# malak29/video-text-detection-system

Measured on AMD Instinct MI355X. Metric: frames/sec (detect+recognize) @720p, 1/2/4/8 MI355X; box IoU vs CPU ref, higher is better.
Workload: dtype f16

## Files before the change

video-text-detection-system_amd/csrc/conv_halo.hip:

```cpp
#include <cstdio>
#include <cstdlib>
#include "vtd_common.h"

namespace {

struct HaloParams {
    const half_t* in;
    const half_t* wgt;
    const float* bias;
    const half_t* res;
    half_t* out;
    int n, h, w, cin, cout;
    int in_hp, in_wp, in_ring, out_hp, out_wp, out_ring, res_hp, res_wp, res_ring;
    int tiles_x, tiles_y, tiles_n, relu;
    unsigned long long* stamps;
    int dbg;
};

template <int N>
__device__ __forceinline__ void hl_wait_vmcnt() {
    asm volatile("s_waitcnt vmcnt(%0)" ::"n"(N) : "memory");
}

template <int BN, int TW>
__global__ __launch_bounds__((BN / 64) * 256) void conv_halo_kernel(const HaloParams p) {
    constexpr int WN = BN / 64, NW = 4 * WN, NT = NW * 64, TH = 256 / TW;
    constexpr int HWD = TW + 2, HROWS = (TH + 2) * HWD, HPIECES = (HROWS + 7) / 8, HBYTES = HPIECES * 1024;
    constexpr int HPW = (HPIECES + NW - 1) / NW;
    constexpr int HPS = (HPW + 7) / 8;
    constexpr int BSTAGE = BN * 128, BPW = BN / 8 / NW;
    constexpr int EPI_ROW = BN * 4 + 16;
    static_assert(BPW == 2, "two weight pieces per wave and K-step");
    extern __shared__ __attribute__((aligned(16))) char smem[];

    const int nchunks = p.cin >> 6;
    const int hb_stride = nchunks > 1 ? HBYTES : 0;
    char* const bring = smem + (nchunks > 1 ? 2 : 1) * HBYTES;

    const int nblk = gridDim.x, b = blockIdx.x;
    const int q8 = nblk >> 3, r8 = nblk & 7, xcd = b & 7;
    int tile = (xcd < r8 ? xcd * (q8 + 1) : r8 * (q8 + 1) + (xcd - r8) * q8) + (b >> 3);
    const int tn = tile % p.tiles_n;
    tile /= p.tiles_n;
    const int tx = tile % p.tiles_x;
    tile /= p.tiles_x;
    const int ty = tile % p.tiles_y;
    const int img = tile / p.tiles_y;
    const int y0 = ty * TH, x0 = tx * TW, n0 = tn * BN;

    const int tid = threadIdx.x, lane = tid & 63;
    const int w = __builtin_amdgcn_readfirstlane(tid >> 6);
    const int lrow = lane >> 3;
    const int K = 9 * p.cin;

// ... 640 lines not shown
    const int grid = total < 256 ? total : 256;
    static const bool want_stamps = [] { const char* e = getenv("VTD_HALO_STAMPS"); return e && e[0] == '1'; }();
    if (want_stamps) {
        HaloParams q = p;
        unsigned long long* dev = nullptr;
        if (hipMalloc(&dev, (size_t)grid * 32) != hipSuccess) return -2204;
        q.stamps = dev;
        hipLaunchKernelGGL((conv3x3_c64_persistent_kernel<TW, RELU, RES>), dim3(grid), dim3(256), lds, stream, q);
        (void)hipStreamSynchronize(stream);
        unsigned long long* h = (unsigned long long*)malloc((size_t)grid * 32);
        (void)hipMemcpy(h, dev, (size_t)grid * 32, hipMemcpyDeviceToHost);
        double a = 0, b = 0, c = 0;
        for (int i = 0; i < grid; ++i) { a += (double)h[4 * i + 1]; b += (double)(h[4 * i + 2] - h[4 * i + 1]); c += (double)(h[4 * i + 3] - h[4 * i + 2]); }
        const double blocks = (double)total / grid;
        fprintf(stderr, "[c64 stamps] res=%d blocks/WG %.1f: per block ticks: issue+wait %.1f  K-loop %.1f  epilogue %.1f\n", (int)RES, blocks,
                a / grid / blocks, b / grid / blocks, c / grid / blocks);
        free(h);
        (void)hipFree(dev);
        return 0;
    }
    const char* duo_env = getenv("VTD_C64_DUO");
    const bool duo = !(duo_env && duo_env[0] == '0');
#ifdef VTD_CONV_EXPERIMENT
    if (duo) {
        HaloParams q = p;
        const char* d = getenv("VTD_C64_DEBUG");
        q.dbg = d ? atoi(d) : 0;
        hipError_t e = hipFuncSetAttribute((const void*)conv3x3_c64_duo_kernel<TW, RELU, RES>, hipFuncAttributeMaxDynamicSharedMemorySize, lds);
        if (e != hipSuccess) return -(int)e;
        hipLaunchKernelGGL((conv3x3_c64_duo_kernel<TW, RELU, RES>), dim3(grid), dim3(512), lds, stream, q);
        return -(int)hipGetLastError();
    }
#endif
    if (duo) {
        static bool attr_duo = false;
        if (!attr_duo) {
            hipError_t e = hipFuncSetAttribute((const void*)conv3x3_c64_duo_kernel<TW, RELU, RES>, hipFuncAttributeMaxDynamicSharedMemorySize, lds);
            if (e != hipSuccess) return -(int)e;
            attr_duo = true;
        }
        hipLaunchKernelGGL((conv3x3_c64_duo_kernel<TW, RELU, RES>), dim3(grid), dim3(512), lds, stream, p);
        return -(int)hipGetLastError();
    }
    hipLaunchKernelGGL((conv3x3_c64_persistent_kernel<TW, RELU, RES>), dim3(grid), dim3(256), lds, stream, p);
    return -(int)hipGetLastError();
}

template <int TW>
int c64_dispatch(const HaloParams& p, hipStream_t stream) {
    if (p.relu) return p.res ? c64_launch<TW, true, true>(p, stream) : c64_launch<TW, true, false>(p, stream);
    return p.res ? c64_launch<TW, false, true>(p, stream) : c64_launch<TW, false, false>(p, stream);
}

template <int BN, int TW>
int halo_launch(const HaloParams& p, hipStream_t stream) {
    constexpr int TH = 256 / TW, HROWS = (TH + 2) * (TW + 2), HBYTES = (HROWS + 7) / 8 * 1024;
    const int nchunks = p.cin / 64;
    const int main_bytes = (nchunks > 1 ? 2 : 1) * HBYTES + 3 * BN * 128;
    const int epi_bytes = 256 * (BN * 4 + 16);
    const int lds = main_bytes > epi_bytes ? main_bytes : epi_bytes;
    if (lds > 160 * 1024) return -2203;
    static int attr_lds = 0;
    if (lds > attr_lds) {
        hipError_t e = hipFuncSetAttribute((const void*)conv_halo_kernel<BN, TW>, hipFuncAttributeMaxDynamicSharedMemorySize, lds);
        if (e != hipSuccess) return -(int)e;
        attr_lds = lds;
    }
    const int grid = p.n * p.tiles_y * p.tiles_x * p.tiles_n;
    static const bool want_stamps = [] { const char* e = getenv("VTD_HALO_STAMPS"); return e && e[0] == '1'; }();
    if (want_stamps) {
        HaloParams q = p;
        unsigned long long* dev = nullptr;
        if (hipMalloc(&dev, (size_t)grid * 32) != hipSuccess) return -2204;
        q.stamps = dev;
        hipLaunchKernelGGL((conv_halo_kernel<BN, TW>), dim3(grid), dim3((BN / 64) * 256), lds, stream, q);
        (void)hipStreamSynchronize(stream);
        unsigned long long* h = (unsigned long long*)malloc((size_t)grid * 32);
        (void)hipMemcpy(h, dev, (size_t)grid * 32, hipMemcpyDeviceToHost);
        double pro = 0, loop = 0, epi = 0;
        unsigned long long t0 = ~0ull, t1 = 0;
        for (int i = 0; i < grid; ++i) {
            pro += (double)(h[4 * i + 1] - h[4 * i]); loop += (double)(h[4 * i + 2] - h[4 * i + 1]); epi += (double)(h[4 * i + 3] - h[4 * i + 2]);
            t0 = h[4 * i] < t0 ? h[4 * i] : t0; t1 = h[4 * i + 3] > t1 ? h[4 * i + 3] : t1;
        }
        fprintf(stderr, "[halo stamps] BN=%d TW=%d cin=%d cout=%d grid=%d: per-WG ticks (100 MHz) prologue %.1f  K-loop %.1f  epilogue %.1f; kernel span %llu ticks\n",
                BN, TW, p.cin, p.cout, grid, pro / grid, loop / grid, epi / grid, t1 - t0);
        free(h);
        (void)hipFree(dev);
        return 0;
    }
    hipLaunchKernelGGL((conv_halo_kernel<BN, TW>), dim3(grid), dim3((BN / 64) * 256), lds, stream, p);
    return -(int)hipGetLastError();
}

}

bool vtd_conv_halo_supported(const ConvParams& c, int* bn_out, int* tw_out) {
    if (c.plist || c.in2 || c.pool_pw || c.stride != 1 || c.kw != 3 || c.K != 9 * c.in_c || (c.in_c & 63)) return false;
    if (c.cin_steps * 64 != c.in_c || c.s_step != c.in_c || c.r_step != c.in_wp * c.in_c || c.k_hi_step != 32) return false;
    if ((c.cout & 63) || c.cout != c.cout_pad || c.out_c != c.cout) return false;
    if (c.flags & ~(EPI_RELU | EPI_RESIDUAL)) return false;
    if ((c.flags & EPI_RESIDUAL) && (c.res_shift || !c.res)) return false;
    if (c.in_y0 < 0 || c.in_x0 != c.in_y0 || c.ho <= 0 || c.wo <= 0 || c.M % (c.ho * c.wo)) return false;
    const int h = c.ho, w = c.wo;
    auto eff = [&](int th, int tw) { return (double)h * w / ((double)((h + th - 1) / th * th) * ((w + tw - 1) / tw * tw)); };
    const double e16 = eff(16, 16), e32 = eff(8, 32);
    const int tw = e16 >= e32 ? 16 : 32;
    if ((tw == 16 ? e16 : e32) < 0.85) return false;
    *tw_out = tw;
    *bn_out = (c.cout % 128 == 0) ? 128 : 64;
    return true;
}

bool vtd_conv_halo_c64_supported(const ConvParams& c, int tw) {
    return c.in_c == 64 && c.cout == 64 && c.wo % tw == 0 && c.ho % (256 / tw) == 0;
}

int vtd_launch_conv_halo(const ConvParams& c, int bn, int tw, hipStream_t stream) {
    HaloParams p;
    p.in = c.in; p.wgt = c.wgt; p.bias = c.bias; p.res = (c.flags & EPI_RESIDUAL) ? c.res : nullptr; p.out = (half_t*)c.out;
    p.h = c.ho; p.w = c.wo; p.n = c.M / (c.ho * c.wo); p.cin = c.in_c; p.cout = c.cout;
    p.in_hp = c.in_hp; p.in_wp = c.in_wp; p.in_ring = c.in_y0 + 1;
    p.out_hp = c.out_hp; p.out_wp = c.out_wp; p.out_ring = c.out_ring;
    p.res_hp = c.res_hp; p.res_wp = c.res_wp; p.res_ring = c.res_ring;
    p.relu = (c.flags & EPI_RELU) ? 1 : 0;
    p.stamps = nullptr;
    p.dbg = 0;
    if (c.in_y0 != c.in_x0 || c.in_y0 < 0 || c.K != 9 * c.in_c || c.out_c != c.cout || p.n <= 0 || (c.in_c & 63) || (c.cout & 63) ||
        (tw != 16 && tw != 32) || c.stride != 1 || c.M != p.n * c.ho * c.wo)
        return -2201;
    if ((int64_t)p.n * c.in_hp * c.in_wp * c.in_c >= (1ll << 31)) return -2202;
    const int th = 256 / tw;
    p.tiles_x = (p.w + tw - 1) / tw; p.tiles_y = (p.h + th - 1) / th; p.tiles_n = bn > 1 ? p.cout / bn : 1;
    if (bn == 2) {
        p.tiles_n = p.cout / 64;
        return tw == 16 ? halo64_launch<16>(p, stream) : halo64_launch<32>(p, stream);
    }
    if (bn == 1) {
        if (p.cin != 64 || p.cout != 64) return -2201;
        p.tiles_n = 1;
        return tw == 16 ? c64_dispatch<16>(p, stream) : c64_dispatch<32>(p, stream);
    }
    if (bn == 64 && tw == 16) return halo_launch<64, 16>(p, stream);
    if (bn == 64 && tw == 32) return halo_launch<64, 32>(p, stream);
    if (bn == 128 && tw == 16) return halo_launch<128, 16>(p, stream);
    if (bn == 128 && tw == 32) return halo_launch<128, 32>(p, stream);
    return -2201;
}
```

video-text-detection-system_amd/csrc/vtd_api.cpp:

```cpp
#include <algorithm>
#include <cmath>
#include <cstdio>
#include <cstdlib>
#include <cstring>
#include <map>
#include <memory>
#include <string>
#include <vector>

#include "../../include/vtd.h"
#include "vtd_common.h"

int vtd_launch_conv(const ConvParams& p, int cfg, hipStream_t stream);
int vtd_conv_num_configs();
bool vtd_conv_config_valid(const ConvParams& p, int cfg);
int vtd_launch_preprocess(const uint8_t* frames, int n, int H, int W, half_t* out, const int* xb, const int* xk, int ksx,
                          const int* yb, const int* yk, int ksy, int max_rows, hipStream_t stream);
int vtd_launch_nchw_to_input(const float* x, half_t* out, int n, hipStream_t stream);
int vtd_launch_maxpool(const TensorDesc& in, const TensorDesc& out, int n, int kh, int kw, int sh, int sw, int pad_h, int pad_w,
                       hipStream_t stream);
void vtd_stem_pool_pack_weights(const float* w_folded, half_t* packed);
int vtd_launch_stem_pool(const TensorDesc& in, const TensorDesc& out, const half_t* w_packed, const float* bias, int n, hipStream_t stream);
extern "C" int vtd_head_entry_halo_steps(int py, int px, int nch1, int* out);
int vtd_launch_head_entry_halo(const ConvParams& c, const int* steps_dev, int nsteps, int big_tiles, hipStream_t stream);
#ifdef VTD_EXPERIMENTAL_CANDIDATES
extern "C" int vtd_head_entry_half_schedule(const int* steps, int nsteps, int* out);
int vtd_launch_head_entry_half(const ConvParams& c, const int* sched_dev, int nsteps, hipStream_t stream);
int vtd_head_entry_pair_tables(int py, int px, int c2ch, int* half_steps, int* plan);
int vtd_launch_head_entry_pair(const ConvParams& c, const int* half_steps_dev, const int* plan_dev, int nh, hipStream_t stream);
#endif
bool vtd_conv_halo_supported(const ConvParams& c, int* bn_out, int* tw_out);
bool vtd_conv_halo_c64_supported(const ConvParams& c, int tw);
int vtd_launch_conv_halo(const ConvParams& c, int bn, int tw, hipStream_t stream);
bool vtd_pointwise128_supported(const ConvParams& c);
int vtd_launch_pointwise128(const ConvParams& c, hipStream_t stream);
void vtd_head_tail_pack_w1(const half_t* w1_gemm, half_t* packed);
void vtd_head_tail_pack_w2(const float* w2, half_t* packed);
int vtd_launch_head_tail(const TensorDesc& in, const half_t* w1, const float* bias1, const half_t* w2, float b2, float* out, int n,
                         hipStream_t stream);

int vtd_launch_crop_resize(const uint8_t* frames, int H, int W, const int32_t* boxes, int ncrops, uint8_t* out, hipStream_t s);
int vtd_launch_crnn_conv1(const uint8_t* in_u8, const float* in_f32, const half_t* w, const float* bias, half_t* out, int n, hipStream_t s);
int vtd_launch_lstm(const half_t* xs, const half_t* whh, half_t* hout, int D, int T, hipStream_t s);
int vtd_launch_ctc_greedy(const float* logits, int n, int T, int V, int ld, const int32_t* id2char, int blank, int apply_softmax,
                          int32_t* out, hipStream_t s);
int vtd_launch_compact_rows(const float* in, float* out, int64_t rows, int V, int ld, hipStream_t s);
int vtd_dbloss_ws_bytes();
int vtd_launch_dbloss(const float* prob, const float* thresh, const float* prob_t, const float* thresh_t, int64_t n, float smooth, double* workspace,
                      float* out4, double* sums5, hipStream_t stream);
int vtd_launch_dbloss_backward(const float* prob, const float* thresh, const float* prob_t, const float* thresh_t, int64_t n, float smooth,
                               const double* sums5, const float* grad_out4, float* grad_prob, float* grad_thresh, hipStream_t stream);
int vtd_launch_binary_counts(const float* pred, const float* target, int64_t n, float threshold, int64_t* counts4, hipStream_t stream);

namespace vtd {

enum : int {
    ERR_ARG = -1100,
    ERR_UNKNOWN_KEY = -1101,
    ERR_SHAPE = -1102,
    ERR_MISSING_KEY = -1103,
    ERR_NOT_FINALIZED = -1104,
    ERR_BATCH = -1105,
    ERR_GEOMETRY = -1106,
    ERR_CAPACITY = -1107,
};

using StateDict = std::map<std::string, std::vector<float>>;

struct DeviceArena {
    std::vector<void*> blocks;
    size_t total = 0;
    int alloc(void** out, size_t bytes, bool zero) {
        void* p = nullptr;
        bytes = (bytes + 255) & ~size_t(255);
        hipError_t e = hipMalloc(&p, bytes);
        if (e != hipSuccess) return -(int)e;
        if (zero) {
            e = hipMemset(p, 0, bytes);
            if (e != hipSuccess) return -(int)e;
        }
        blocks.push_back(p);
        total += bytes;
        *out = p;
        return 0;
    }
// ... 46 lines not shown
    const float* bias_tab = nullptr;
    bool dual = false;
    int in2_mul = 1, in2_shr = 0;
    int pool_pw = 0;
};

struct Op {
    enum Kind { CONV, POOL, FINAL, STEMPOOL, HEADTAIL, BORDER } kind;
    ConvOp conv;
    TensorDesc pin, pout;
    int pk[6] = {0, 0, 0, 0, 0, 0};
    const float* fw = nullptr;
    float fbias = 0.f;
    int final_slot = 0;
    const half_t* spw = nullptr;
    const float* spb = nullptr;
    const half_t* htw1 = nullptr;
    const half_t* htw2 = nullptr;
};

static void fill_conv_params(const ConvOp& c, int n, ConvParams& p) {
    std::memset(&p, 0, sizeof(p));
    p.in = c.in.ptr; p.wgt = c.w; p.k_hi_step = c.k_hi_step; p.cin_steps = c.cin_steps; p.kw = c.kw; p.s_step = c.s_step; p.r_step = c.r_step; p.bias = c.bias;
    p.res = c.has_res ? c.res.ptr : nullptr;
    p.out = (c.flags & (EPI_OUT_F32 | EPI_OUT_F16)) ? c.out_f32 : (void*)c.out.ptr;
    p.M = n * c.ho * c.wo; p.K = c.K; p.cout = c.cout; p.cout_pad = c.cout_pad;
    p.ho = c.ho; p.wo = c.wo;
    p.in_hp = c.in.hp; p.in_wp = c.in.wp; p.in_c = c.in.c; p.in_y0 = c.in_y0; p.in_x0 = c.in_x0; p.stride = c.stride;
    p.out_hp = c.out.hp; p.out_wp = c.out.wp; p.out_c = c.out.c; p.out_ring = c.out.ring;
    p.res_hp = c.res.hp; p.res_wp = c.res.wp; p.res_ring = c.res.ring; p.res_shift = c.res_shift;
    p.ps_cout = c.ps_cout; p.flags = c.flags; p.ldc = c.ldc;
    p.seg_cols = c.seg_cols;
    for (int i = 0; i < 3; ++i) { p.seg_out[i] = c.seg_out[i]; p.seg_ldc[i] = c.seg_ldc[i]; }
    p.head_w = c.head_w; p.head_b = c.head_b; p.prob_out = (float*)c.out_f32;
    if (c.plist) {
        p.plist = c.plist; p.tile_combo = c.tile_combo; p.tiles_per_img = c.tiles_per_img;
        p.plist_b = c.plist_b; p.tile_combo_b = c.tile_combo_b; p.tiles_per_img_b = c.tiles_per_img_b;
        p.in2 = c.in2.ptr; p.in2_hp = c.in2.hp; p.in2_wp = c.in2.wp; p.in2_c = c.in2.c; p.in2_ring = c.in2.ring;
        p.seg1_steps = c.seg1_steps; p.cin_steps2 = c.cin_steps2; p.kw2 = c.kw2; p.s_step2 = c.s_step2; p.r_step2 = c.r_step2;
        p.bias_tab = c.bias_tab; p.img_h = c.img_h; p.img_w = c.img_w;
        p.M = n * c.tiles_per_img * 128;
    }
    p.pool_pw = c.pool_pw;
    if (c.dual) {
        p.in2 = c.in2.ptr; p.in2_hp = c.in2.hp; p.in2_wp = c.in2.wp; p.in2_c = c.in2.c; p.in2_ring = c.in2.ring;
        p.in2_mul = c.in2_mul; p.in2_shr = c.in2_shr;
        p.seg1_steps = c.seg1_steps; p.cin_steps2 = c.cin_steps2; p.kw2 = 1; p.s_step2 = 0; p.r_step2 = 0;
    }
}

static const int kHaloCfg = 100;
static const int kHaloC64Cfg = 101;
static const int kHalo64Cfg = 104;
static const int kHeadEntryHalo256Cfg = 103;
static const int kHeadEntryPairCfg = 105;
static const int kPointwiseCfg = 106;
static const int kHeadEntryHalfCfg = 107;
static const int kHeadEntryHaloCfg = 102;
static bool halo_enabled() {
    const char* e = std::getenv("VTD_HALO_CONV");
    return !(e && e[0] == '0');
}

static int pick_tile_height(const ConvParams& p, int table_cfg) {
    if (const char* e = std::getenv("VTD_TILE_HEIGHT_MODEL"); e && e[0] == '0') return table_cfg;
    if (std::getenv("VTD_FORCE_CONV_CFG")) return table_cfg;
    static const struct { int cfg, bm, bn; double eff; } family[5] = {{0, 256, 128, 1.0}, {14, 256, 128, 1.04}, {13, 272, 128, 0.92}, {12, 208, 128, 0.80},
                                                                      {15, 256, 256, 1.07}};
    auto cost_of = [&](int cfg) -> double {
        for (const auto& k : family)
            if (k.cfg == cfg) {
                if (!vtd_conv_config_valid(p, k.cfg)) return 0.0;
                const int64_t tiles = (int64_t)((p.M + k.bm - 1) / k.bm) * (p.cout_pad / k.bn);
                return (double)((tiles + 255) / 256) * k.bm * k.bn / k.eff;
            }
        return 0.0;
    };
    int best = table_cfg;
    double best_cost = cost_of(table_cfg);
    if (best_cost == 0.0) return table_cfg;
    const double keep = best_cost * 0.94;
    double other_cost = keep;
    for (const auto& k : family) {
        if (k.cfg == table_cfg) continue;
        const double c = cost_of(k.cfg);
        if (c > 0.0 && c < other_cost) { other_cost = c; best = k.cfg; }
    }
    (void)best_cost;
    return best;
}

static int launch_conv_op(const ConvOp& c, int n, hipStream_t s, int cfg = -1, float* prob_out = nullptr) {
    ConvParams p;
    fill_conv_params(c, n, p);
    if (prob_out) p.prob_out = prob_out;
#ifdef VTD_EXPERIMENTAL_CANDIDATES
    if (cfg == kHeadEntryPairCfg) {
        if (!c.hp_half_steps || !c.tile_combo_border) return ERR_GEOMETRY;
        return vtd_launch_head_entry_pair(p, c.hp_half_steps, c.hp_plan, c.hp_nh, s);
    }
    if (cfg == kHeadEntryHalfCfg) {
        if (!c.hh_sched || !c.tile_combo_border) return ERR_GEOMETRY;
        return vtd_launch_head_entry_half(p, c.hh_sched, c.he_nsteps, s);
    }
#else
    if (cfg == kHeadEntryPairCfg || cfg == kHeadEntryHalfCfg) return ERR_GEOMETRY;
#endif
    if (cfg == kHeadEntryHaloCfg || cfg == kHeadEntryHalo256Cfg) {
        if (!c.he_steps || !c.tile_combo_border) return ERR_GEOMETRY;
        return vtd_launch_head_entry_halo(p, c.he_steps, c.he_nsteps, cfg == kHeadEntryHalo256Cfg ? 1 : 0, s);
    }
    if (cfg == kHaloCfg || cfg == kHaloC64Cfg || cfg == kHalo64Cfg) {
        int bn = 0, tw = 0;
        if (!vtd_conv_halo_supported(p, &bn, &tw)) return ERR_GEOMETRY;
        return vtd_launch_conv_halo(p, cfg == kHaloC64Cfg ? 1 : cfg == kHalo64Cfg ? 2 : bn, tw, s);
    }
    if (cfg == kPointwiseCfg) return vtd_launch_pointwise128(p, s);
    if (!c.plist && (cfg == 0 || cfg == 12 || cfg == 13 || cfg == 14 || cfg == 15)) cfg = pick_tile_height(p, cfg);
    return vtd_launch_conv(p, cfg, s);
}

static int launch_border_tiles(const ConvOp& c, int n, hipStream_t s) {
    if (!c.tile_combo_border || c.tiles_border <= 0) return ERR_GEOMETRY;
    ConvParams pb;
    fill_conv_params(c, n, pb);
    pb.tile_combo = c.tile_combo_border; pb.tiles_per_img = c.tiles_border; pb.M = n * c.tiles_border * 128;
    pb.plist_b = nullptr; pb.tile_combo_b = nullptr; pb.tiles_per_img_b = 0;
    return vtd_launch_conv(pb, 9, s);
}

static int autotune_conv(const ConvOp& c, int n, hipStream_t s, int* best_cfg) {
    ConvParams p;
    fill_conv_params(c, n, p);
    hipEvent_t e0, e1;
    VTD_HIP_CHECK(hipEventCreate(&e0));
    VTD_HIP_CHECK(hipEventCreate(&e1));
    float best = 1e30f;
    int best_id = -1, rc = 0;
    if (p.plist) {
        const char* fc = std::getenv("VTD_FORCE_CLASSED_CFG");
        if (fc && (vtd_conv_config_valid(p, std::atoi(fc)) || ((std::atoi(fc) == kHeadEntryHaloCfg || std::atoi(fc) == kHeadEntryHalo256Cfg) && c.he_steps) ||
                   (std::atoi(fc) == kHeadEntryHalfCfg && c.hh_sched) ||
                   (std::atoi(fc) == kHeadEntryPairCfg && c.hp_half_steps))) {
            (void)hipEventDestroy(e0);
            (void)hipEventDestroy(e1);
            *best_cfg = std::atoi(fc);
            return 0;
        }
    }
    for (int cfg = 0; cfg < vtd_conv_num_configs() && !rc; ++cfg) {
        if (!vtd_conv_config_valid(p, cfg)) continue;
        if ((rc = vtd_launch_conv(p, cfg, s))) break;
        (void)hipEventRecord(e0, s);
        for (int rep = 0; rep < 3 && !rc; ++rep) rc = vtd_launch_conv(p, cfg, s);
        (void)hipEventRecord(e1, s);
        if (hipEventSynchronize(e1) != hipSuccess) { rc = ERR_ARG; break; }
        float ms = 0.f;
        (void)hipEventElapsedTime(&ms, e0, e1);
        if (ms < best) { best = ms; best_id = cfg; }
    }
    if (!rc && p.plist && c.he_steps && halo_enabled()) {
        const float best_gathered = best;
        for (int variant = 0; variant < 4 && !rc; ++variant) {
            if (variant == 2 && !c.hp_half_steps) continue;
            if (variant == 3 && !c.hh_sched) continue;
            const int vcfg = variant == 3 ? kHeadEntryHalfCfg : variant == 2 ? kHeadEntryPairCfg : variant ? kHeadEntryHalo256Cfg : kHeadEntryHaloCfg;
            auto both = [&]() { int r = launch_conv_op(c, n, s, vcfg); return r ? r : launch_border_tiles(c, n, s); };
            if ((rc = both())) break;
            float ms = 1e30f;
            for (int round = 0; round < 2 && !rc; ++round) {
                (void)hipEventRecord(e0, s);
                for (int rep = 0; rep < 4 && !rc; ++rep) rc = both();
                (void)hipEventRecord(e1, s);
                if (hipEventSynchronize(e1) != hipSuccess) rc = ERR_ARG;
                float t = 0.f;
                (void)hipEventElapsedTime(&t, e0, e1);
                ms = t * 0.75f < ms ? t * 0.75f : ms;
            }
            if (const char* v = std::getenv("VTD_AUTOTUNE_VERBOSE"); v && v[0] == '1')
                std::fprintf(stderr, "[autotune] head entry variant %d: %.1f us per launch incl. border tiles (best so far %.1f, cfg %d)\n", vcfg,
                             ms / 3.f * 1e3f, best / 3.f * 1e3f, best_id);
            (void)best_gathered;
            if (!rc && ms < best) { best = ms; best_id = vcfg; }
        }
    }
    if (!rc && vtd_pointwise128_supported(p)) {
        if (!(rc = vtd_launch_pointwise128(p, s))) {
            (void)hipEventRecord(e0, s);
            for (int rep = 0; rep < 3 && !rc; ++rep) rc = vtd_launch_pointwise128(p, s);
            (void)hipEventRecord(e1, s);
            if (hipEventSynchronize(e1) != hipSuccess) rc = ERR_ARG;
            float ms = 0.f;
            (void)hipEventElapsedTime(&ms, e0, e1);
            if (!rc && ms < best) { best = ms; best_id = kPointwiseCfg; }
        }
    }
    int hbn = 0, htw = 0;
    if (!rc && halo_enabled() && vtd_conv_halo_supported(p, &hbn, &htw)) {
        const char* force = std::getenv("VTD_FORCE_HALO");
        if (force && (force[0] == '1' || force[0] == '2' || force[0] == '3')) best = 1e30f;
        bool pinned = false;
        for (int variant = 0; variant < 3 && !rc; ++variant) {
            if (variant == 1 && !vtd_conv_halo_c64_supported(p, htw)) continue;
            const int bn = variant == 1 ? 1 : variant == 2 ? 2 : hbn;
            if ((rc = vtd_launch_conv_halo(p, bn, htw, s))) break;
            (void)hipEventRecord(e0, s);
            for (int rep = 0; rep < 3 && !rc; ++rep) rc = vtd_launch_conv_halo(p, bn, htw, s);
            (void)hipEventRecord(e1, s);
            if (hipEventSynchronize(e1) != hipSuccess) rc = ERR_ARG;
            float ms = 0.f;
            (void)hipEventElapsedTime(&ms, e0, e1);
            const int vid = variant == 1 ? kHaloC64Cfg : variant == 2 ? kHalo64Cfg : kHaloCfg;
            const bool pin = (variant == 1 && force && force[0] == '2') || (variant == 2 && force && force[0] == '3');
            if (!rc && !pinned && (ms < best || pin)) { best = ms; best_id = vid; pinned = pin; }
        }
    }
    (void)hipEventDestroy(e0);
    (void)hipEventDestroy(e1);
    *best_cfg = best_id;
    if (const char* v = std::getenv("VTD_AUTOTUNE_VERBOSE"); v && v[0] == '1')
        std::fprintf(stderr, "[autotune] M=%d N=%d K=%d%s -> cfg %d (%.1f us per launch)\n", p.M, p.cout, p.K, p.plist ? " classed" : "", best_id,
                     best / 3.f * 1e3f);
    return rc;
}

static bool autotune_enabled() {
    const char* e = std::getenv("VTD_AUTOTUNE");
    return !(e && e[0] == '0');
}

struct ResampleAxis {
    int ksize = 0;
    std::vector<int> bounds, kk;
};
static ResampleAxis pillow_axis(int in_size, int out_size) {
    ResampleAxis a;
    const double scale = (double)in_size / out_size;
    const double fscale = scale < 1.0 ? 1.0 : scale;
    const double support = fscale;
    a.ksize = (int)std::ceil(support) * 2 + 1;
    a.bounds.assign(2 * (size_t)out_size, 0);
    a.kk.assign((size_t)out_size * a.ksize, 0);
    std::vector<double> pre(a.ksize);
    for (int xx = 0; xx < out_size; ++xx) {
        const double center = (xx + 0.5) * scale, ss = 1.0 / fscale;
        int xmin = (int)(center - support + 0.5);
        if (xmin < 0) xmin = 0;
        int xmax = (int)(center + support + 0.5);
        if (xmax > in_size) xmax = in_size;
        xmax -= xmin;
        double ww = 0.0;
        for (int x = 0; x < xmax; ++x) {
            double t = (x + xmin - center + 0.5) * ss;
            if (t < 0) t = -t;
            const double wv = t < 1.0 ? 1.0 - t : 0.0;
            pre[x] = wv;
            ww += wv;
        }
        for (int x = 0; x < xmax; ++x) {
            const double v = ww != 0.0 ? pre[x] / ww : pre[x];
            a.kk[(size_t)xx * a.ksize + x] = v < 0 ? (int)(-0.5 + v * (1 << 22)) : (int)(0.5 + v * (1 << 22));
        }
        a.bounds[2 * xx] = xmin;
        a.bounds[2 * xx + 1] = xmax;
    }
    return a;
}

struct PreTables {
    int *xb = nullptr, *xk = nullptr, *yb = nullptr, *yk = nullptr;
    int ksx = 0, ksy = 0, max_rows = 0;
};

}

using namespace vtd;

namespace vtd {
struct ModelBase {
    StateDict sd;
    DeviceArena arena;
    std::map<std::string, int> tuning;
    bool tuning_measured = false;
    int alloc_tensor(TensorDesc& t) {
        void* p = nullptr;
        int rc = arena.alloc(&p, (size_t)tensor_elems(t) * sizeof(half_t), true);
        t.ptr = (half_t*)p;
        return rc;
    }
    const std::vector<float>* get(const std::string& k, size_t numel) const {
        auto it = sd.find(k);
        if (it == sd.end() || it->second.size() != numel) return nullptr;
        return &it->second;
    }
};

static std::string conv_signature(const ConvOp& c) {
    char buf[192];
    int len = std::snprintf(buf, sizeof buf, "conv|in%dx%dx%d|out%dx%d|co%d|K%d|s%d|f%x|r%d|c%d", c.in.h, c.in.w, c.in.c, c.ho, c.wo, c.cout, c.K,
                            c.stride, (unsigned)c.flags, c.has_res ? 1 + c.res_shift : 0, c.plist ? 1 : 0);
    if (c.dual) len += std::snprintf(buf + len, sizeof buf - len, "|x%dm%ds%d", c.in2.c, c.in2_mul, c.in2_shr);
    if (c.pool_pw) std::snprintf(buf + len, sizeof buf - len, "|p2x%d", c.pool_pw);
    return buf;
}

static bool config_valid_for(const ConvOp& c, int n, int cfg) {
    ConvParams p;
    fill_conv_params(c, n, p);
    if (cfg == kHeadEntryPairCfg) return p.plist && c.hp_half_steps && c.tile_combo_border;
    if (cfg == kHeadEntryHalfCfg) return p.plist && c.hh_sched && c.tile_combo_border;
    if (cfg == kHeadEntryHaloCfg || cfg == kHeadEntryHalo256Cfg) return p.plist && c.he_steps && c.tile_combo_border;
    if (cfg == kHaloCfg || cfg == kHaloC64Cfg || cfg == kHalo64Cfg) {
        int bn = 0, tw = 0;
        if (!vtd_conv_halo_supported(p, &bn, &tw)) return false;
        return cfg != kHaloC64Cfg || vtd_conv_halo_c64_supported(p, tw);
    }
    if (cfg == kPointwiseCfg) return vtd_pointwise128_supported(p);
    return cfg >= 0 && cfg < vtd_conv_num_configs() && vtd_conv_config_valid(p, cfg);
}

static int choose_config(ModelBase* m, const ConvOp& c, int n, hipStream_t s, int* cfg) {
    const std::string key = conv_signature(c) + "|n" + std::to_string(n);
    auto it = m->tuning.find(key);
    const bool forced = std::getenv("VTD_FORCE_CLASSED_CFG") || std::getenv("VTD_FORCE_HALO");
    if (const char* fc = std::getenv("VTD_FORCE_CONV_CFG"); fc && !c.plist && config_valid_for(c, n, std::atoi(fc))) {
        *cfg = std::atoi(fc);
        return 0;
    }
    if (const char* fp = std::getenv("VTD_FORCE_POINTWISE"); fp && fp[0] == '1' && config_valid_for(c, n, kPointwiseCfg)) {
        *cfg = kPointwiseCfg;
        return 0;
    }
    if (!forced && it != m->tuning.end() && config_valid_for(c, n, it->second)) {
        *cfg = it->second;
        return 0;
    }
    *cfg = -1;
    if (!autotune_enabled()) return 0;
    int rc = autotune_conv(c, n, s, cfg);
    if (!rc && *cfg >= 0) {
        m->tuning[key] = *cfg;
        m->tuning_measured = true;
    }
    return rc;
}

static int set_tuning_text(ModelBase* m, const char* text) {
    if (!m || !text) return ERR_ARG;
    const char* p = text;
    while (*p) {
        const char* eol = std::strchr(p, '\n');
        std::string line = eol ? std::string(p, eol) : std::string(p);
        p = eol ? eol + 1 : p + line.size();
        if (line.empty() || line[0] == '#') continue;
        const size_t sp = line.find_last_of(" \t");
        if (sp == std::string::npos || sp + 1 >= line.size()) return ERR_ARG;
        char* end = nullptr;
        const long v = std::strtol(line.c_str() + sp + 1, &end, 10);
        if (!end || *end != 0) return ERR_ARG;
        size_t ke = sp;
        while (ke > 0 && (line[ke - 1] == ' ' || line[ke - 1] == '\t')) --ke;
        m->tuning[line.substr(0, ke)] = (int)v;
    }
    return 0;
}

static int64_t get_tuning_text(const ModelBase* m, char* buf, int64_t cap) {
// ... 965 lines not shown
}

int vtd_detector_num_ops(const vtd_detector* d) { return d ? (int)d->ops.size() : 0; }

int vtd_detector_set_tuning(vtd_detector* d, const char* table_text) {
    if (!d) return ERR_ARG;
    int rc = set_tuning_text(d, table_text);
    if (!rc) d->tuned.clear();
    return rc;
}

int64_t vtd_detector_get_tuning(const vtd_detector* d, char* buf, int64_t capacity) { return get_tuning_text(d, buf, capacity); }

int vtd_detector_tuning_measured(const vtd_detector* d) { return d && d->tuning_measured ? 1 : 0; }

int vtd_detector_get_profile(vtd_detector* d, int op_index, char* name, int name_cap, double* total_ms, int64_t* calls,
                             double* total_macs, vtd_stream stream) {
    if (!d || op_index < 0 || op_index >= (int)d->ops.size() || !name || name_cap < 32 || !total_ms || !calls || !total_macs)
        return ERR_ARG;
    if (!d->ev_spans.empty()) {
        hipError_t e = hipStreamSynchronize((hipStream_t)stream);
        if (e != hipSuccess) return -(int)e;
        for (auto& sp : d->ev_spans) {
            float ms = 0.f;
            e = hipEventElapsedTime(&ms, sp.second.first, sp.second.second);
            if (e != hipSuccess) return -(int)e;
            d->prof_ms[sp.first] += ms;
            d->prof_calls[sp.first] += 1;
        }
        d->ev_spans.clear();
        d->ev_used = 0;
    }
    const Op& o = d->ops[op_index];
    if (o.kind == Op::CONV) {
        const ConvOp& c = o.conv;
        static const char* kTile[] = {"256,128,s3", "128,128,s2", "128,128,s3", "256,64,s2", "256,64,s3", "128,64,s2", "128,64,s3",
                                      "64,256,s2", "128,64,s2,classed", "128,64,s3,classed", "256,64,s2,classed", "256,64,s3,classed", "208,128,s3", "272,128,s3", "256,128,s3,16w", "256,256,s2", "128,64,s6"};
        int cfg = -1;
        if (!d->tuned.empty()) cfg = d->tuned.rbegin()->second[op_index];
        if (cfg == kHeadEntryPairCfg)
            std::snprintf(name, name_cap, "head_entry_pair M/img=%d N=%d K=%d (lateral+smooth+head conv composed; border classes in the "
                          "next slot)", c.ho * c.wo, c.cout, c.K);
        else if (cfg == kHeadEntryHalfCfg)
            std::snprintf(name, name_cap, "head_entry_half M/img=%d N=%d K=%d (lateral+smooth+head conv composed, half halos two steps ahead; border classes in the "
                          "next slot)", c.ho * c.wo, c.cout, c.K);
        else if (cfg == kHeadEntryHalo256Cfg)
            std::snprintf(name, name_cap, "head_entry_halo256 M/img=%d N=%d K=%d (lateral+smooth+head conv composed; border classes in the "
                          "next slot)", c.ho * c.wo, c.cout, c.K);
        else if (cfg == kHeadEntryHaloCfg)
            std::snprintf(name, name_cap, "head_entry_halo M/img=%d N=%d K=%d (lateral+smooth+head conv composed; border classes in the "
                          "next slot)", c.ho * c.wo, c.cout, c.K);
        else if (cfg == kPointwiseCfg)
            std::snprintf(name, name_cap, "pointwise128 1x1%s streaming M/img=%d N=%d K=%d", c.has_res ? "+top-down add" : "", c.ho * c.wo, c.cout, c.K);
        else if (cfg == kHaloCfg || cfg == kHaloC64Cfg || cfg == kHalo64Cfg)
            std::snprintf(name, name_cap, "conv_halo%s 3x3 M/img=%d N=%d K=%d", cfg == kHaloC64Cfg ? "_c64_persistent" : cfg == kHalo64Cfg ? "64" : "",
                          c.ho * c.wo, c.cout, c.K);
        else
            std::snprintf(name, name_cap, "conv_igemm<%s> M/img=%d N=%d K=%d%s", (cfg >= 0 && cfg < 17) ? kTile[cfg] : "default",
                          c.ho * c.wo, c.cout, c.K, c.plist ? " (lateral+smooth+head conv composed)" : "");
    } else if (o.kind == Op::POOL) {
        std::snprintf(name, name_cap, "maxpool %dx%d/s%d", o.pk[0], o.pk[1], o.pk[2]);
    } else if (o.kind == Op::BORDER) {
        std::snprintf(name, name_cap, "conv_igemm<128,64,s3,classed> border classes of the composed head entry (%d tiles/img)", o.conv.tiles_border);
    } else if (o.kind == Op::HEADTAIL) {
        std::snprintf(name, name_cap, "head_tail ConvT1+BN+ReLU+ConvT2+sigmoid fused M/img=%d N=256 K=64", o.conv.ho * o.conv.wo);
    } else if (o.kind == Op::STEMPOOL) {
        std::snprintf(name, name_cap, "stem_pool conv7x7/s2+BN+ReLU+maxpool3x3/s2 fused M/img=%d N=64 K=147", 320 * 320);
    } else {
        std::snprintf(name, name_cap, "conv_igemm<64,256,s2> ConvT1+ConvT2+sigmoid fused M/img=%d", o.conv.ho * o.conv.wo);
    }
    const bool have = d->prof_ms.size() == d->ops.size();
    *total_ms = have ? d->prof_ms[op_index] : 0.0;
    *calls = have ? d->prof_calls[op_index] : 0;
    *total_macs = have ? d->prof_macs[op_index] : 0.0;
    return 0;
}

int vtd_detector_read_tap(vtd_detector* d, const char* name, int n, float* host_out, int64_t capacity, vtd_stream stream) {
    if (!d || !name || !host_out) return ERR_ARG;
    if (!d->finalized) return ERR_NOT_FINALIZED;
    auto it = d->taps.find(name);
    if (it == d->taps.end()) return ERR_UNKNOWN_KEY;
    const TensorDesc& t = it->second;
    if (n <= 0 || n > t.n) return ERR_BATCH;
    const int creal = (std::string(name) == "input") ? 3 : t.c;
    if (capacity < (int64_t)n * creal * t.h * t.w) return ERR_CAPACITY;
    return read_tensor_nchw(t, n, creal, host_out, (hipStream_t)stream);
}

int64_t vtd_detector_macs_per_frame(const vtd_detector* d) { return d ? d->macs : 0; }

}

namespace vtd {

static int build_recognizer_graph(vtd_recognizer* r) {
    const int D = r->max_crops;
    int rc;
    auto new_tensor = [&](int h, int w, int c, int ring, TensorDesc& t) {
        t = make_desc(D, h, w, c, ring, ring);
        return r->alloc_tensor(t);
    };
    void* p = nullptr;
    if ((rc = r->arena.alloc(&p, (size_t)D * 32 * 128 * 3, true))) return rc;
    r->resized = (uint8_t*)p;
    {
        Fold f;
        if ((rc = fold_bn(r, "cnn.1", "cnn.0.bias", 64, f))) return rc;
// ... 229 lines not shown
```

Baseline: 12050.

## Add persistent 128-channel 3x3 halo conv kernel with weight ring pipeline

Adds a persistent 512-thread kernel for 128-in/128-out 3x3 convolutions. Each block loops over 16-wide spatial tiles, streams per-tap weight slices through an R-stage LDS ring, and prefetches the next tile's input halo while computing the current one. Explicit vmcnt waits are derived from a compile-time load plan. The kernel is registered as a new autotune variant, so it runs only where it times faster. The cost is more code and reliance on hand-counted wait values being correct.

```diff
diff --git a/video-text-detection-system_amd/csrc/conv_halo.hip b/video-text-detection-system_amd/csrc/conv_halo.hip
--- a/video-text-detection-system_amd/csrc/conv_halo.hip
+++ b/video-text-detection-system_amd/csrc/conv_halo.hip
@@ -1,5 +1,6 @@
 #include <cstdio>
 #include <cstdlib>
+#include <utility>
 #include "vtd_common.h"
 
 namespace {
@@ -746,6 +747,219 @@
     return p.res ? c64_launch<TW, false, true>(p, stream) : c64_launch<TW, false, false>(p, stream);
 }
 
+template <int HPW, int JR, int R, bool RES>
+struct C128Plan {
+    static constexpr int halo_at(int tap) {
+        int n = 0;
+        for (int k = tap; tap < 4 && k < HPW; k += 4) ++n;
+        return n;
+    }
+    static constexpr int extra(int u) {
+        u = ((u % 18) + 18) % 18;
+        return halo_at(u % 9) + ((RES && u == 9) ? JR : 0);
+    }
+    static constexpr int after_res() {
+        int n = 0;
+        for (int u = 10; u < 18; ++u) n += 2 + extra(u);
+        return n;
+    }
+    static constexpr int newer(int t) {
+        int n = extra(t - R + 1);
+        for (int u = t - R + 2; u < t; ++u) n += 2 + extra(u);
+        return n;
+    }
+};
+
+template <int... Is, class F>
+__device__ __forceinline__ void c128_unroll(std::integer_sequence<int, Is...>, F&& f) {
+    (f(std::integral_constant<int, Is>{}), ...);
+}
+
+template <int TH, int R, bool RELU, bool RES>
+__global__ __launch_bounds__(512, 1) void conv3x3_c128_persistent_kernel(const HaloParams p) {
+    constexpr int TW = 16, JR = TH / 2, HWD = TW + 2, HROWS = (TH + 2) * HWD, HPIECES = (HROWS + 7) / 8, HBYTES = HPIECES * 1024;
+    constexpr int HPW = (HPIECES + 7) / 8;
+    constexpr int SBYTES = 128 * 128;
+    using Plan = C128Plan<HPW, JR, R, RES>;
+    static_assert(TH % 2 == 0 && HPW <= 8, "block shape");
+    static_assert(Plan::newer(0) == 2 * (R - 2), "the prologue issues exactly the loads step 0's wait counts");
+    static_assert(R * SBYTES + 2 * HBYTES + 1024 <= 160 * 1024, "LDS budget");
+    extern __shared__ __attribute__((aligned(16))) char smem[];
+    char* const ring = smem;
+    char* const hbuf = smem + R * SBYTES;
+
+    const int tid = threadIdx.x, lane = tid & 63;
+    const int w = __builtin_amdgcn_readfirstlane(tid >> 6);
+    const int wp = w & 1, wc = w >> 1;
+    const int lrow = lane >> 3, fr = lane & 15, fq = lane >> 4;
+    const int tiles_per_img = p.tiles_x * p.tiles_y, total = p.n * tiles_per_img;
+
+    const int grid = gridDim.x, b = blockIdx.x;
+    const int q8 = grid >> 3, r8 = grid & 7, xcd = b & 7;
+    const int vb = (xcd < r8 ? xcd * (q8 + 1) : r8 * (q8 + 1) + (xcd - r8) * q8) + (b >> 3);
+    const int nmine = (total - vb + grid - 1) / grid;
+    auto tile_coords = [&](int t, int& img, int& y0, int& x0) {
+        img = t / tiles_per_img;
+        const int r = t - img * tiles_per_img, ty = r / p.tiles_x;
+        y0 = ty * TH;
+        x0 = (r - ty * p.tiles_x) * TW;
+    };
+
+    floatx4 bias0 = *(const floatx4*)(p.bias + wc * 32 + fq * 8), bias1 = *(const floatx4*)(p.bias + wc * 32 + fq * 8 + 4);
+    asm volatile("" : "+v"(bias0), "+v"(bias1));
+
+    int bsrc[2];
+#pragma unroll
+    for (int i = 0; i < 2; ++i) {
+        const int r = (w + 8 * i) * 8 + lrow;
+        const int cout = 32 * (r >> 5) + 8 * ((r & 15) >> 2) + 4 * ((r >> 4) & 1) + (r & 3);
+        bsrc[i] = cout * 1152 + ((lane & 7) ^ ((r >> 1) & 7)) * 8;
+    }
+    auto issue_b = [&](int chunk, int tap, int stage) {
+#pragma unroll
+        for (int i = 0; i < 2; ++i)
+            __builtin_amdgcn_global_load_lds((const VTD_AS1 void*)(p.wgt + bsrc[i] + tap * 128 + chunk * 64),
+                                             (VTD_AS3 void*)(ring + stage * SBYTES + (w + 8 * i) * 1024), 16, 0, 0);
+    };
+    int hrel[HPW];
+#pragma unroll
+    for (int k = 0; k < HPW; ++k) {
+        int row = (w + 8 * k) * 8 + lrow;
+        row = row < HROWS ? row : HROWS - 1;
+        const int hy = row / HWD, hx = row - hy * HWD;
+        hrel[k] = (hy * p.in_wp + hx) * 128 + ((lane & 7) ^ (hx & 6)) * 8;
+    }
+    auto issue_halo = [&](int k, int img, int y0, int x0, int chunk) {
+        const half_t* base = p.in + ((int64_t)(img * p.in_hp + y0 - 1 + p.in_ring) * p.in_wp + x0 - 1 + p.in_ring) * 128 + chunk * 64;
+        const int piece = w + 8 * k;
+        char* dst = piece < HPIECES ? hbuf + chunk * HBYTES + piece * 1024 : hbuf + 2 * HBYTES;
+        __builtin_amdgcn_global_load_lds((const VTD_AS1 void*)(base + hrel[k]), (VTD_AS3 void*)dst, 16, 0, 0);
+    };
+
+    const int a_lane_off = (wp * JR * HWD + fr) * 128;
+    const int b_lane_off = (wc * 32 + fr) * 128;
+    const int bswz = (fr >> 1) & 7;
+
+    int img, y0, x0;
+    tile_coords(vb, img, y0, x0);
+#pragma unroll
+    for (int k = 0; k < HPW; ++k) issue_halo(k, img, y0, x0, 0);
+#pragma unroll
+    for (int s = 0; s < R - 1; ++s) issue_b(s / 9, s % 9, s);
+
+    int blk = vb;
+    for (int kb = 0; kb < nmine; ++kb, blk += grid) {
+        int nimg = img, ny0 = y0, nx0 = x0;
+        if (kb + 1 < nmine) tile_coords(blk + grid, nimg, ny0, nx0);
+        const int sbase = (18 % R == 0) ? 0 : (kb * 18) % R;
+
+        floatx4 acc[2][JR];
+#pragma unroll
+        for (int j = 0; j < JR; ++j) { acc[0][j] = bias0; acc[1][j] = bias1; }
+        half8 rv[JR];
+
+        c128_unroll(std::make_integer_sequence<int, 18>{}, [&](auto tc) {
+            constexpr int t = decltype(tc)::value, chunk = t / 9, tap = t % 9;
+            hl_wait_vmcnt<Plan::newer(t)>();
+            __builtin_amdgcn_s_barrier();
+            {
+                constexpr int tn = (t + R - 1) % 18;
+                issue_b(tn / 9, tn % 9, (sbase + t + R - 1) % R);
+            }
+            if constexpr (tap < 4) {
+#pragma unroll
+                for (int k = tap; k < HPW; k += 4) {
+                    if (chunk == 0) issue_halo(k, img, y0, x0, 1);
+                    else issue_halo(k, nimg, ny0, nx0, 0);
+                }
+            }
+            if constexpr (RES && t == 9) {
+#pragma unroll
+                for (int j = 0; j < JR; ++j) {
+                    const int y = y0 + wp * JR + j, x = x0 + fr;
+                    const half_t* src = p.res + ((int64_t)(img * p.res_hp + y + p.res_ring) * p.res_wp + x + p.res_ring) * 128 + wc * 32 + fq * 8;
+                    asm volatile("global_load_dwordx4 %0, %1, off" : "=v"(rv[j]) : "v"(src) : "memory");
+                }
+            }
+            constexpr int dy = tap / 3, dx = tap % 3;
+            const char* sb = ring + ((sbase + t) % R) * SBYTES + b_lane_off;
+            const char* hb = hbuf + chunk * HBYTES + a_lane_off + (dy * HWD + dx) * 128;
+#pragma unroll
+            for (int kk = 0; kk < 2; ++kk) {
+                half8 af[JR], bf[2];
+                const int ach = ((fq + 4 * kk) ^ ((fr + dx) & 6)) << 4;
+#pragma unroll
+                for (int j = 0; j < JR; ++j) af[j] = *(const half8*)(hb + j * HWD * 128 + ach);
+#pragma unroll
+                for (int i = 0; i < 2; ++i) bf[i] = *(const half8*)(sb + i * 2048 + (((fq + 4 * kk) ^ bswz) << 4));
+#pragma unroll
+                for (int i = 0; i < 2; ++i)
+#pragma unroll
+                    for (int j = 0; j < JR; ++j) acc[i][j] = __builtin_amdgcn_mfma_f32_16x16x32_f16(bf[i], af[j], acc[i][j], 0, 0, 0);
+            }
+        });
+
+        if constexpr (RES) {
+            hl_wait_vmcnt<Plan::after_res()>();
+#pragma unroll
+            for (int j = 0; j < JR; ++j) asm volatile("" : "+v"(rv[j]));
+        }
+        half_t* obase = p.out + ((int64_t)(img * p.out_hp + y0 + p.out_ring) * p.out_wp + x0 + p.out_ring) * 128 + wc * 32 + fq * 8;
+#pragma unroll
+        for (int j = 0; j < JR; ++j) {
+            half8 hv;
+#pragma unroll
+            for (int e = 0; e < 8; ++e) {
+                float v = acc[e >> 2][j][e & 3];
+                if (RES) v += (float)rv[j][e];
+                hv[e] = (half_t)(RELU ? fmaxf(v, 0.f) : v);
+            }
+            *(half8*)(obase + ((wp * JR + j) * p.out_wp + fr) * 128) = hv;
+        }
+        img = nimg; y0 = ny0; x0 = nx0;
+    }
+    hl_wait_vmcnt<0>();
+}
+
+template <int TH, int R, bool RELU, bool RES>
+int c128_launch_t(const HaloParams& p, hipStream_t stream) {
+    constexpr int HBYTES = ((TH + 2) * 18 + 7) / 8 * 1024;
+    constexpr int lds = R * 128 * 128 + 2 * HBYTES + 1024;
+    static_assert(lds <= 160 * 1024, "LDS budget");
+    static bool attr_done = false;
+    if (!attr_done) {
+        hipError_t e = hipFuncSetAttribute((const void*)conv3x3_c128_persistent_kernel<TH, R, RELU, RES>,
+                                           hipFuncAttributeMaxDynamicSharedMemorySize, lds);
+        if (e != hipSuccess) return -(int)e;
+        attr_done = true;
+    }
+    const int total = p.n * p.tiles_y * p.tiles_x;
+    const int rounds = (total + 255) / 256;
+    const int grid = (total + rounds - 1) / rounds;
+    hipLaunchKernelGGL((conv3x3_c128_persistent_kernel<TH, R, RELU, RES>), dim3(grid), dim3(512), lds, stream, p);
+    return -(int)hipGetLastError();
+}
+
+template <int TH, int R>
+int c128_dispatch(const HaloParams& p, hipStream_t stream) {
+    if (p.relu) return p.res ? c128_launch_t<TH, R, true, true>(p, stream) : c128_launch_t<TH, R, true, false>(p, stream);
+    return p.res ? c128_launch_t<TH, R, false, true>(p, stream) : c128_launch_t<TH, R, false, false>(p, stream);
+}
+
+int c128_block_height(int n, int h, int w) {
+    if (n <= 0 || h <= 0 || w <= 0 || w % 16) return 0;
+    static const int kHeights[2] = {10, 8};
+    int best = 0;
+    long best_cost = 0;
+    for (int th : kHeights) {
+        if (h % th) continue;
+        const long blocks = (long)n * (h / th) * (w / 16);
+        const long cost = (blocks + 255) / 256 * (th + 2);
+        if (!best || cost < best_cost) { best = th; best_cost = cost; }
+    }
+    return best;
+}
+
 template <int BN, int TW>
 int halo_launch(const HaloParams& p, hipStream_t stream) {
     constexpr int TH = 256 / TW, HROWS = (TH + 2) * (TW + 2), HBYTES = (HROWS + 7) / 8 * 1024;
@@ -808,6 +1022,14 @@
 
 bool vtd_conv_halo_c64_supported(const ConvParams& c, int tw) {
     return c.in_c == 64 && c.cout == 64 && c.wo % tw == 0 && c.ho % (256 / tw) == 0;
+}
+
+bool vtd_conv_halo_c128_supported(const ConvParams& c) {
+    if (c.in_c != 128 || c.cout != 128 || c.cout_pad != 128 || c.out_c != 128 || c.K != 1152 || c.stride != 1 || c.kw != 3) return false;
+    if (c.ho <= 0 || c.wo <= 0 || c.M % (c.ho * c.wo)) return false;
+    const int ring = c.in_y0 + 1;
+    if (ring < 1 || c.in_x0 != c.in_y0 || c.in_hp < c.ho + ring + 1 || c.in_wp < c.wo + ring + 1) return false;
+    return c128_block_height(c.M / (c.ho * c.wo), c.ho, c.wo) > 0;
 }
 
 int vtd_launch_conv_halo(const ConvParams& c, int bn, int tw, hipStream_t stream) {
@@ -830,6 +1052,13 @@
         p.tiles_n = p.cout / 64;
         return tw == 16 ? halo64_launch<16>(p, stream) : halo64_launch<32>(p, stream);
     }
+    if (bn == 3) {
+        if (!vtd_conv_halo_c128_supported(c)) return -2201;
+        const int th = c128_block_height(p.n, p.h, p.w);
+        p.tiles_x = p.w / 16; p.tiles_y = p.h / th; p.tiles_n = 1;
+        if (th == 10) return c128_dispatch<10, 6>(p, stream);
+        return c128_dispatch<8, 6>(p, stream);
+    }
     if (bn == 1) {
         if (p.cin != 64 || p.cout != 64) return -2201;
         p.tiles_n = 1;
diff --git a/video-text-detection-system_amd/csrc/vtd_api.cpp b/video-text-detection-system_amd/csrc/vtd_api.cpp
--- a/video-text-detection-system_amd/csrc/vtd_api.cpp
+++ b/video-text-detection-system_amd/csrc/vtd_api.cpp
@@ -31,6 +31,7 @@
 #endif
 bool vtd_conv_halo_supported(const ConvParams& c, int* bn_out, int* tw_out);
 bool vtd_conv_halo_c64_supported(const ConvParams& c, int tw);
+bool vtd_conv_halo_c128_supported(const ConvParams& c);
 int vtd_launch_conv_halo(const ConvParams& c, int bn, int tw, hipStream_t stream);
 bool vtd_pointwise128_supported(const ConvParams& c);
 int vtd_launch_pointwise128(const ConvParams& c, hipStream_t stream);
@@ -183,6 +184,7 @@
 static const int kHaloCfg = 100;
 static const int kHaloC64Cfg = 101;
 static const int kHalo64Cfg = 104;
+static const int kHaloC128Cfg = 108;
 static const int kHeadEntryHalo256Cfg = 103;
 static const int kHeadEntryPairCfg = 105;
 static const int kPointwiseCfg = 106;
@@ -241,10 +243,11 @@
         if (!c.he_steps || !c.tile_combo_border) return ERR_GEOMETRY;
         return vtd_launch_head_entry_halo(p, c.he_steps, c.he_nsteps, cfg == kHeadEntryHalo256Cfg ? 1 : 0, s);
     }
-    if (cfg == kHaloCfg || cfg == kHaloC64Cfg || cfg == kHalo64Cfg) {
+    if (cfg == kHaloCfg || cfg == kHaloC64Cfg || cfg == kHalo64Cfg || cfg == kHaloC128Cfg) {
         int bn = 0, tw = 0;
         if (!vtd_conv_halo_supported(p, &bn, &tw)) return ERR_GEOMETRY;
-        return vtd_launch_conv_halo(p, cfg == kHaloC64Cfg ? 1 : cfg == kHalo64Cfg ? 2 : bn, tw, s);
+        if (cfg == kHaloC128Cfg && !vtd_conv_halo_c128_supported(p)) return ERR_GEOMETRY;
+        return vtd_launch_conv_halo(p, cfg == kHaloC64Cfg ? 1 : cfg == kHalo64Cfg ? 2 : cfg == kHaloC128Cfg ? 3 : bn, tw, s);
     }
     if (cfg == kPointwiseCfg) return vtd_launch_pointwise128(p, s);
     if (!c.plist && (cfg == 0 || cfg == 12 || cfg == 13 || cfg == 14 || cfg == 15)) cfg = pick_tile_height(p, cfg);
@@ -329,11 +332,12 @@
     int hbn = 0, htw = 0;
     if (!rc && halo_enabled() && vtd_conv_halo_supported(p, &hbn, &htw)) {
         const char* force = std::getenv("VTD_FORCE_HALO");
-        if (force && (force[0] == '1' || force[0] == '2' || force[0] == '3')) best = 1e30f;
+        if (force && (force[0] == '1' || force[0] == '2' || force[0] == '3' || force[0] == '4')) best = 1e30f;
         bool pinned = false;
-        for (int variant = 0; variant < 3 && !rc; ++variant) {
+        for (int variant = 0; variant < 4 && !rc; ++variant) {
             if (variant == 1 && !vtd_conv_halo_c64_supported(p, htw)) continue;
-            const int bn = variant == 1 ? 1 : variant == 2 ? 2 : hbn;
+            if (variant == 3 && !vtd_conv_halo_c128_supported(p)) continue;
+            const int bn = variant == 1 ? 1 : variant == 2 ? 2 : variant == 3 ? 3 : hbn;
             if ((rc = vtd_launch_conv_halo(p, bn, htw, s))) break;
             (void)hipEventRecord(e0, s);
             for (int rep = 0; rep < 3 && !rc; ++rep) rc = vtd_launch_conv_halo(p, bn, htw, s);
@@ -341,8 +345,9 @@
             if (hipEventSynchronize(e1) != hipSuccess) rc = ERR_ARG;
             float ms = 0.f;
             (void)hipEventElapsedTime(&ms, e0, e1);
-            const int vid = variant == 1 ? kHaloC64Cfg : variant == 2 ? kHalo64Cfg : kHaloCfg;
-            const bool pin = (variant == 1 && force && force[0] == '2') || (variant == 2 && force && force[0] == '3');
+            const int vid = variant == 1 ? kHaloC64Cfg : variant == 2 ? kHalo64Cfg : variant == 3 ? kHaloC128Cfg : kHaloCfg;
+            const bool pin = (variant == 1 && force && force[0] == '2') || (variant == 2 && force && force[0] == '3') ||
+                             (variant == 3 && force && force[0] == '4');
             if (!rc && !pinned && (ms < best || pin)) { best = ms; best_id = vid; pinned = pin; }
         }
     }
@@ -441,9 +446,10 @@
     if (cfg == kHeadEntryPairCfg) return p.plist && c.hp_half_steps && c.tile_combo_border;
     if (cfg == kHeadEntryHalfCfg) return p.plist && c.hh_sched && c.tile_combo_border;
     if (cfg == kHeadEntryHaloCfg || cfg == kHeadEntryHalo256Cfg) return p.plist && c.he_steps && c.tile_combo_border;
-    if (cfg == kHaloCfg || cfg == kHaloC64Cfg || cfg == kHalo64Cfg) {
+    if (cfg == kHaloCfg || cfg == kHaloC64Cfg || cfg == kHalo64Cfg || cfg == kHaloC128Cfg) {
         int bn = 0, tw = 0;
         if (!vtd_conv_halo_supported(p, &bn, &tw)) return false;
+        if (cfg == kHaloC128Cfg) return vtd_conv_halo_c128_supported(p);
         return cfg != kHaloC64Cfg || vtd_conv_halo_c64_supported(p, tw);
     }
     if (cfg == kPointwiseCfg) return vtd_pointwise128_supported(p);
@@ -1515,8 +1521,9 @@
                           "next slot)", c.ho * c.wo, c.cout, c.K);
         else if (cfg == kPointwiseCfg)
             std::snprintf(name, name_cap, "pointwise128 1x1%s streaming M/img=%d N=%d K=%d", c.has_res ? "+top-down add" : "", c.ho * c.wo, c.cout, c.K);
-        else if (cfg == kHaloCfg || cfg == kHaloC64Cfg || cfg == kHalo64Cfg)
-            std::snprintf(name, name_cap, "conv_halo%s 3x3 M/img=%d N=%d K=%d", cfg == kHaloC64Cfg ? "_c64_persistent" : cfg == kHalo64Cfg ? "64" : "",
+        else if (cfg == kHaloCfg || cfg == kHaloC64Cfg || cfg == kHalo64Cfg || cfg == kHaloC128Cfg)
+            std::snprintf(name, name_cap, "conv_halo%s 3x3 M/img=%d N=%d K=%d",
+                          cfg == kHaloC64Cfg ? "_c64_persistent" : cfg == kHalo64Cfg ? "64" : cfg == kHaloC128Cfg ? "_c128_persistent" : "",
                           c.ho * c.wo, c.cout, c.K);
         else
             std::snprintf(name, name_cap, "conv_igemm<%s> M/img=%d N=%d K=%d%s", (cfg >= 0 && cfg < 17) ? kTile[cfg] : "default",
```

After: 12250, median of 6. 1.6% higher.
